# tyh666/News-Recommendation-MIND

Hardware: AMD Instinct MI355X
Metric: impressions/sec (train) + candidates scored/sec (eval), NRMS MIND-large 1/8 GPU (higher is better)
Workload: dtype f32; 1 GPU; NRMS train step: MHA news encoder + MHA user encoder, H=384, 12 heads, V=30522 word table (trainable), dropout 0.2, Adam; launch=hipGraph replay of the whole step, global_batch=32, per_gpu_batch=32, candidates=5, history=50, seq_len=30, parallelism=dp1

## Files before the change

include/newsrec_hip.h:

```cpp
#ifndef NEWSREC_HIP_H
#define NEWSREC_HIP_H

#include <stdint.h>

#ifdef __cplusplus
extern "C" {
#endif

typedef struct ihipStream_t* hipStream_t;

const char* nr_build_hash(void);


enum nr_rows_map {
  NR_ROWS_PLAIN = 0,
  NR_ROWS_GATHER = 1,
  NR_ROWS_CONV3 = 2
};

enum nr_layout {
  NR_KCONTIG = 0,
  NR_MNCONTIG = 1
};

// ... 134 lines not shown
                    int64_t ld_dout, float* dqk, int64_t ld_dqk, float* dv_out, int64_t ld_dv,
                    float* dbias_k, float* dbias_v, hipStream_t stream);

int nr_mha_pool_fwd(const float* y, int64_t ldy, const int64_t* yrows, const void* mask,
                    int32_t mask_dtype, int64_t nseq,
                    int32_t L, int32_t heads, int32_t dk, int32_t dv, const float* gamma,
                    const float* beta, float eps, float p_drop, uint64_t seed, uint64_t offset,
                    const uint64_t* rng, const float* q, float* news, int64_t ldn, float* zout,
                    int64_t ldz, float* oout, int64_t ldo, float* stats, float* probs,
                    int32_t prec, hipStream_t stream);

int nr_mha_pool_bwd(const float* y, int64_t ldy, const int64_t* yrows, const void* mask,
                    int32_t mask_dtype, int64_t nseq,
                    int32_t L, int32_t heads, int32_t dk, int32_t dv, const float* gamma,
                    const float* beta, float p_drop, uint64_t seed, uint64_t offset,
                    const uint64_t* rng, const float* q, const float* stats, const float* probs,
                    const float* dnews,
                    int64_t ldn, const float* dz, int64_t lddz, const float* o, int64_t ldo,
                    float* dob, int64_t lddob, float* dy, int64_t lddy,
                    float* dbias, float* dq, float* dgamma, float* dbeta, float* ws,
                    int32_t ws_copies, const int32_t* seg_off, int64_t dyu_row0, int64_t dy_rows,
                    uint32_t* dsto, int32_t prec, hipStream_t stream);


int nr_attn_pool_fwd(const float* x, int64_t ldx, const float* key, int64_t ldk, const float* q,
                     const void* mask, int32_t mask_dtype, const float* gamma, const float* beta,
                     float eps, float p_drop, uint64_t seed, uint64_t offset, const uint64_t* rng,
                     int64_t nseq, int32_t L, int32_t D, float scale, float* out, int64_t ldo,
                     float* zout,
                     int64_t ldz, float* stats, float* probs, hipStream_t stream);

int nr_attn_pool_bwd(const float* x, int64_t ldx, const float* key, int64_t ldk, const float* q,
                     const void* mask, int32_t mask_dtype, const float* gamma, const float* beta,
                     float p_drop, uint64_t seed, uint64_t offset, const uint64_t* rng,
                     int64_t nseq, int32_t L, int32_t D, float scale, const float* stats,
                     const float* probs,
                     const float* dout, int64_t lddo, const float* dz, int64_t lddz, float* dx,
                     int64_t lddx, float* dk, int64_t lddk, int32_t key_tanh, float* dq,
                     float* dgamma, float* dbeta, hipStream_t stream);

int nr_seq_pool_fwd(const float* x, int64_t ldx, const float* key, int64_t ldk, const float* q, int32_t qn,
                    const void* mask, int32_t mask_dtype, int64_t nseq, int32_t L, int32_t D, float scale,
                    float* out, int64_t ldo, float* probs, hipStream_t stream);

int nr_seq_pool_bwd(const float* x, int64_t ldx, const float* key, int64_t ldk, const float* q, int32_t qn,
                    const void* mask, int32_t mask_dtype, int64_t nseq, int32_t L, int32_t D, float scale,
// ... 248 lines not shown
```

news-recommendation-mind_amd/csrc/mha_pool.hip:

```cpp
#include "common.h"
#include "../../include/newsrec_hip.h"
#include <stdlib.h>

#include "mfma_planes.h"

namespace {

struct MPArgs {
  const float* y; int64_t ldy;
  const int64_t* yrows;
  const void* mask; int mask_dt;
  int64_t nseq; int L; int heads;
  float scale_attn, scale_pool;
  const float* gamma; const float* beta; float eps;
  float p_drop; uint64_t seed; uint64_t offset;
  uint32_t dkey, dthresh;
  const uint64_t* rng;
  const float* q;
  float* news; int64_t ldn;
  float* zout; int64_t ldz;
  float* stats; float* probs;
  const float* dz; int64_t lddz;
  float* dy; int64_t lddy;
  const int32_t* seg_off; int64_t dyu_row0;
// ... 41 lines not shown
__device__ __forceinline__ uint32_t row_byte_off(const MPArgs& g, int64_t tok) {
  return (uint32_t)((g.yrows ? g.yrows[tok] : tok) * g.ldy * 4);
}

__device__ __forceinline__ void stage_rows(const MPArgs& g, int64_t seq) {
  extern __shared__ uint32_t nr_mp_rows[];
  const int tid = threadIdx.x;
  if (tid < 32) nr_mp_rows[tid] = row_byte_off(g, seq * g.L + (tid < g.L ? tid : 0));
  __syncthreads();
}

__device__ __forceinline__ float drop_scale(const MPArgs& g, int64_t elem) {
  if (g.p_drop <= 0.f) return 1.f;
  return nr_dropout_keep(g.dkey, (uint32_t)elem, g.dthresh) ? 1.f / (1.f - g.p_drop) : 0.f;
}

__device__ __forceinline__ uint64_t token_bits(const MPArgs& g, int64_t seq) {
  const int lane = threadIdx.x & 63;
  const bool m = lane < g.L && nr_mask_at(g.mask, g.mask_dt, seq * g.L + lane);
  return __ballot(m);
}

template <int DK, int NP>
__device__ __forceinline__ void load_krow(const MPArgs& g, int64_t seq, int head, float (&a)[DK / 2]) {
  const int lane = threadIdx.x & 63, c = lane & 31, h = lane >> 5;
  constexpr int HK = DK / 2;
  if constexpr (NP > 0) {
    const bool ok = c < g.L;
    const float* kr = yrow(g, ok ? c : 0) + head * DK + 8 * h;
#pragma unroll
    for (int t = 0; t < DK / 16; ++t) {
#pragma unroll
      for (int q4 = 0; q4 < 2; ++q4) {
        const float4 v = *reinterpret_cast<const float4*>(kr + 16 * t + 4 * q4);
        float* d = a + 8 * t + 4 * q4;
        d[0] = ok ? v.x : 0.f; d[1] = ok ? v.y : 0.f; d[2] = ok ? v.z : 0.f; d[3] = ok ? v.w : 0.f;
      }
    }
  } else {
    const bool ok = c < g.L;
    const float* kr = yrow(g, ok ? c : 0) + head * DK + 4 * h;
#pragma unroll
    for (int s = 0; s < HK; s += 4) {
      const float4 v = *reinterpret_cast<const float4*>(kr + 2 * s);
      a[s] = ok ? v.x : 0.f; a[s + 1] = ok ? v.y : 0.f; a[s + 2] = ok ? v.z : 0.f; a[s + 3] = ok ? v.w : 0.f;
    }
  }
}

template <int DK, int NP>
__device__ __forceinline__ void stage_kblock(const float (&a)[DK / 2], int kb, float* tw) {
  const int lane = threadIdx.x & 63, c = lane & 31, h = lane >> 5;
  if constexpr (NP > 0) {
#pragma unroll
    for (int t = 2 * kb; t < 2 * kb + 2; ++t)
#pragma unroll
      for (int u = 0; u < 8; ++u) tw[c * 33 + 16 * t + 8 * h + u - 32 * kb] = a[8 * t + u];
  } else {
#pragma unroll
    for (int m = 4 * kb; m < 4 * kb + 4; ++m)
#pragma unroll
      for (int q = 0; q < 4; ++q) tw[c * 33 + 8 * m + 4 * h + q - 32 * kb] = a[4 * m + q];
  }
}

template <int DK, int NP>
__device__ __forceinline__ void head_probs_from(const MPArgs& g, uint64_t bits, const float (&a)[DK / 2],
                                                float (&p)[16]) {
  const int lane = threadIdx.x & 63, c = lane & 31, h = lane >> 5;
  constexpr int HK = DK / 2;
  f32x16 S;
#pragma unroll
  for (int r = 0; r < 16; ++r) S[r] = 0.f;
  if constexpr (NP == 0) {
#pragma unroll
    for (int s = 0; s < HK; ++s) S = __builtin_amdgcn_mfma_f32_32x32x2f32(a[s], a[s], S, 0, 0, 0);
  } else {
#pragma unroll
    for (int t = 0; t < DK / 16; ++t) {
      const Planes<NP> pk = planes8<NP>(a + 8 * t);
      mfma_x<NP>(S, pk, pk);
    }
  }
  const bool mj = (bits >> c) & 1ull;
  float mx = -INFINITY;
#pragma unroll
  for (int r = 0; r < 16; ++r) {
    const bool keep = mj && ((bits >> crow(r, h)) & 1ull);
    p[r] = keep ? S[r] * g.scale_attn : -INFINITY;
    mx = fmaxf(mx, p[r]);
  }
  mx = fmaxf(mx, __shfl_xor(mx, 32, 64));
// ... 243 lines not shown
      b += red[(ww * 3 + 1) * H + d];
      q += red[(ww * 3 + 2) * H + d];
    }
    atomicAdd(g.ws ? grad_slot(g, d) : &g.dgamma[d], a);
    atomicAdd(g.ws ? grad_slot(g, H + d) : &g.dbeta[d], b);
    atomicAdd(g.ws ? grad_slot(g, 2 * H + d) : &g.dq[d], q);
  }
  __syncthreads();
}

template <int DV>
struct DoSource {
  const float* base;
  int64_t ld;
  int L;
  bool global;
  __device__ __forceinline__ float at(int l, int col) const {
    if (!global) return base[l * ld + col];
    const float v = ld_off(base, 4u * (uint32_t)((l < L ? l : 0) * (int)ld + col));
    return l < L ? v : 0.f;
  }
};

template <int DK, int DV, int NP>
__device__ __forceinline__ void head_bwd(const MPArgs& g, int64_t seq, int head, uint64_t bits, float* tw,
                                         const DoSource<DV>& dO, float (&cs)[DV / 32 + DK / 32],
                                         const uint32_t* dsto) {
  const int lane = threadIdx.x & 63, c = lane & 31, h = lane >> 5;
  const int nq = g.heads * DK;

  float p[16];
  float ka[DK / 2];
  load_krow<DK, NP>(g, seq, head, ka);
  head_probs_from<DK, NP>(g, bits, ka, p);
  __builtin_amdgcn_sched_barrier(0);
  {
#pragma unroll
    for (int r = 0; r < 16; ++r) tw[c * 33 + crow(r, h)] = p[r];
    wave_lds_fence();
    float pt[16];
#pragma unroll
    for (int s = 0; s < 16; ++s) pt[s] = tw[crow(s, h) * 33 + c];
    wave_lds_fence();
#pragma unroll
    for (int vb = 0; vb < DV / 32; ++vb) {
      float bo[16];
#pragma unroll
      for (int s = 0; s < 16; ++s) bo[s] = dO.at(crow(s, h), vb * 32 + c);
      f32x16 acc;
#pragma unroll
      for (int r = 0; r < 16; ++r) acc[r] = 0.f;
      mfma16<NP>(acc, pt, bo);
      float sum = 0.f;
#pragma unroll
      for (int r = 0; r < 16; ++r) {
        const int i = crow(r, h);
        if (i < g.L && dsto[i] != ~0u) st_off(g.dy, dsto[i] + 4u * (uint32_t)(nq + head * DV + vb * 32 + c), acc[r]);
        sum += acc[r];
      }
      cs[vb] += sum;
      __builtin_amdgcn_sched_barrier(0);
    }
  }
  float dsv[16];
  {
    f32x16 dpt;
#pragma unroll
    for (int r = 0; r < 16; ++r) dpt[r] = 0.f;
    constexpr int HV = DV / 2;
    const bool rv = c < g.L;
    if constexpr (NP == 0) {
      const float* vrr = yrow(g, rv ? c : 0) + nq + head * DV + 4 * h;
#pragma unroll
      for (int s = 0; s < HV; s += 4) {
        float4 v4 = *reinterpret_cast<const float4*>(vrr + 2 * s);
        if (!rv) v4 = make_float4(0.f, 0.f, 0.f, 0.f);
        const int col = 4 * h + 2 * s;
        dpt = __builtin_amdgcn_mfma_f32_32x32x2f32(v4.x, dO.at(c, col), dpt, 0, 0, 0);
        dpt = __builtin_amdgcn_mfma_f32_32x32x2f32(v4.y, dO.at(c, col + 1), dpt, 0, 0, 0);
        dpt = __builtin_amdgcn_mfma_f32_32x32x2f32(v4.z, dO.at(c, col + 2), dpt, 0, 0, 0);
        dpt = __builtin_amdgcn_mfma_f32_32x32x2f32(v4.w, dO.at(c, col + 3), dpt, 0, 0, 0);
      }
    } else {
      const float* vrr = yrow(g, rv ? c : 0) + nq + head * DV + 8 * h;
#pragma unroll
      for (int t = 0; t < DV / 16; ++t) {
        float va[8], oa[8];
#pragma unroll
        for (int q4 = 0; q4 < 2; ++q4) {
          const float4 v4 = *reinterpret_cast<const float4*>(vrr + 16 * t + 4 * q4);
          va[4 * q4] = rv ? v4.x : 0.f; va[4 * q4 + 1] = rv ? v4.y : 0.f;
          va[4 * q4 + 2] = rv ? v4.z : 0.f; va[4 * q4 + 3] = rv ? v4.w : 0.f;
        }
#pragma unroll
        for (int u = 0; u < 8; ++u) oa[u] = dO.at(c, 16 * t + 8 * h + u);
        mfma_x<NP>(dpt, planes8<NP>(va), planes8<NP>(oa));
      }
    }
    float rs = 0.f;
#pragma unroll
    for (int r = 0; r < 16; ++r) rs = fmaf(p[r], dpt[r], rs);
    rs += __shfl_xor(rs, 32, 64);
#pragma unroll
    for (int r = 0; r < 16; ++r) dsv[r] = p[r] * (dpt[r] - rs) * g.scale_attn;
  }
  __builtin_amdgcn_sched_barrier(0);
#pragma unroll
  for (int r = 0; r < 16; ++r) tw[c * 33 + crow(r, h)] = dsv[r];
  wave_lds_fence();
#pragma unroll
  for (int r = 0; r < 16; ++r) dsv[r] += tw[crow(r, h) * 33 + c];
  wave_lds_fence();
#pragma unroll
  for (int kb = 0; kb < DK / 32; ++kb) {
    stage_kblock<DK, NP>(ka, kb, tw);
    wave_lds_fence();
    float bk[16];
#pragma unroll
    for (int s = 0; s < 16; ++s) bk[s] = tw[crow(s, h) * 33 + c];
    wave_lds_fence();
    f32x16 acc;
#pragma unroll
    for (int r = 0; r < 16; ++r) acc[r] = 0.f;
    mfma16<NP>(acc, dsv, bk);
    float sum = 0.f;
#pragma unroll
    for (int r = 0; r < 16; ++r) {
      const int j = crow(r, h);
      if (j < g.L && dsto[j] != ~0u) st_off(g.dy, dsto[j] + 4u * (uint32_t)(head * DK + kb * 32 + c), acc[r]);
      sum += acc[r];
    }
    cs[DV / 32 + kb] += sum;
    __builtin_amdgcn_sched_barrier(0);
  }
}

template <int DK, int DV>
__device__ __forceinline__ void flush_dbias(const MPArgs& g, int head, float (&cs)[DV / 32 + DK / 32]) {
  const int lane = threadIdx.x & 63, c = lane & 31, h = lane >> 5;
  const int nq = g.heads * DK;
#pragma unroll
  for (int i = 0; i < DV / 32 + DK / 32; ++i) {
    const float v = cs[i] + __shfl_xor(cs[i], 32, 64);
    const int col = i < DV / 32 ? nq + head * DV + i * 32 + c : head * DK + (i - DV / 32) * 32 + c;
    if (h == 0) atomicAdd(g.ws ? grad_slot(g, 3 * (int64_t)g.heads * DV + col) : &g.dbias[col], v);
    cs[i] = 0.f;
  }
}

template <int DK, int DV, int NH64, int NP, bool SAVED>
__global__ __launch_bounds__(384) void mha_pool_bwd_kernel(MPArgs g) {
  if (g.rng) g.dkey = nr_dropout_key(g.rng[0], g.rng[1] + g.offset);
  extern __shared__ __attribute__((aligned(16))) float sm[];
  constexpr int H = NH64 * 64;
  constexpr int SO = H + 1;
  const int nw = blockDim.x >> 6;
  float* os = sm + 32;
// ... 135 lines not shown
    if (lane == 0) {
      float4* rc = reinterpret_cast<float4*>(g.dob + row * g.lddob);
      rc[0] = make_float4(g.stats[2 * row], rstd, sg, sgx);
      rc[1] = make_float4(dsl, pl, 0.f, 0.f);
    }
  }
#pragma unroll
  for (int k = 0; k < NH64; ++k) {
    red[w][0][lane + 64 * k] = dgam[k];
    red[w][1][lane + 64 * k] = dbet[k];
    red[w][2][lane + 64 * k] = dqp[k];
  }
  __syncthreads();
  float* ogam = g.ws ? grad_slot(g, 0) : g.dgamma;
  float* obet = g.ws ? grad_slot(g, H) : g.dbeta;
  float* oq = g.ws ? grad_slot(g, 2 * H) : g.dq;
  for (int d = tid; d < H; d += 256) {
    atomicAdd(&ogam[d], (red[0][0][d] + red[1][0][d]) + (red[2][0][d] + red[3][0][d]));
    atomicAdd(&obet[d], (red[0][1][d] + red[1][1][d]) + (red[2][1][d] + red[3][1][d]));
    atomicAdd(&oq[d], (red[0][2][d] + red[1][2][d]) + (red[2][2][d] + red[3][2][d]));
  }
}

constexpr int HB_TITLES = 1;

template <int DK, int DV, int NP>
__global__ __launch_bounds__(256, 4) void mha_head_bwd_kernel(MPArgs g) {
  if (g.rng) g.dkey = nr_dropout_key(g.rng[0], g.rng[1] + g.offset);
  extern __shared__ __attribute__((aligned(16))) float sm[];
  const int lane = threadIdx.x & 63, w = threadIdx.x >> 6, nw = blockDim.x >> 6;
  const int head = blockIdx.y * nw + w;
  if (head >= g.heads) return;
  uint32_t* rows = reinterpret_cast<uint32_t*>(sm) + 32 * w;
  uint32_t* dsts = reinterpret_cast<uint32_t*>(sm) + 32 * nw + 32 * w;
  float* tw = sm + 64 * nw + w * 32 * 33;
  float* dot = sm + 64 * nw + nw * 32 * 33 + w * 32 * (DV + 1);
  float cs[DV / 32 + DK / 32];
#pragma unroll
  for (int i = 0; i < DV / 32 + DK / 32; ++i) cs[i] = 0.f;
  const int64_t s0 = (int64_t)blockIdx.x * HB_TITLES;
#pragma unroll 1
  for (int64_t seq = s0; seq < s0 + HB_TITLES && seq < g.nseq; ++seq) {
    const uint32_t roff = lane < 32 ? row_byte_off(g, seq * g.L + (lane < g.L ? lane : 0)) : 0u;
    const uint64_t bits = token_bits(g, seq);
    uint32_t doff = ~0u;
    if (lane < g.L) doff = g.dsto ? g.dsto[seq * g.L + lane] : (uint32_t)((seq * g.L + lane) * g.lddy * 4);
    constexpr int F4 = DV / 4;
    constexpr int PER = 32 * F4 / 64;
    static_assert(64 % F4 == 0, "a lane keeps its four columns in every row it loads");
    float4 v[PER], ra[PER], rb[PER];
    const int col0 = head * DV + 4 * (lane % F4);
    {
      const float* src = g.o + (seq * g.L) * g.ldo + head * DV;
#pragma unroll
      for (int i = 0; i < PER; ++i) {
        const int e = lane + 64 * i, r = e / F4, c4 = e % F4;
        const int rr = r < g.L ? r : 0;
        v[i] = *reinterpret_cast<const float4*>(
            reinterpret_cast<const char*>(src) + 4u * (uint32_t)(rr * (int)g.ldo + 4 * c4));
        const float4* rc = reinterpret_cast<const float4*>(g.dob + (seq * g.L + rr) * g.lddob);
        ra[i] = rc[0];
        rb[i] = rc[1];
      }
    }
    float gm[4], qd[4], dn[4];
#pragma unroll
    for (int j = 0; j < 4; ++j) {
      gm[j] = g.gamma[col0 + j];
      qd[j] = g.q[col0 + j];
      dn[j] = g.news[seq * g.ldn + col0 + j];
    }
    {
      const bool drop = g.p_drop > 0.f;
      const float dsc = drop ? 1.f / (1.f - g.p_drop) : 1.f;
      const uint32_t Hc = (uint32_t)(g.heads * DV);
#pragma unroll
      for (int i = 0; i < PER; ++i) {
        const int r = (lane + 64 * i) / F4;
        const int64_t row = seq * g.L + (r < g.L ? r : 0);
        float o[4] = {v[i].x, v[i].y, v[i].z, v[i].w}, d[4];
#pragma unroll
        for (int j = 0; j < 4; ++j) {
          const uint32_t col = (uint32_t)(col0 + j);
          const bool keep = !drop || nr_dropout_keep(g.dkey, (uint32_t)row * Hc + col, g.dthresh);
          const float dzv = g.dz ? g.dz[row * g.lddz + col] : 0.f;
          const float xh = (o[j] - ra[i].x) * ra[i].y;
          d[j] = ln_row_dO(xh, ra[i].y, ra[i].z, ra[i].w, rb[i].y, rb[i].x, dn[j], qd[j], gm[j], dzv,
                           keep ? dsc : 0.f);
        }
        v[i] = r < g.L ? make_float4(d[0], d[1], d[2], d[3]) : make_float4(0.f, 0.f, 0.f, 0.f);
      }
    }
    if (lane < 32) {
      rows[lane] = roff;
      dsts[lane] = doff;
    }
#pragma unroll
    for (int i = 0; i < PER; ++i) {
      const int e = lane + 64 * i, r = e / F4, c4 = e % F4;
      float* d = dot + r * (DV + 1) + 4 * c4;
      d[0] = v[i].x; d[1] = v[i].y; d[2] = v[i].z; d[3] = v[i].w;
    }
    wave_lds_fence();
    DoSource<DV> dO{dot, DV + 1, g.L, false};
    head_bwd<DK, DV, NP>(g, seq, head, bits, tw, dO, cs, dsts);
    wave_lds_fence();
  }
  flush_dbias<DK, DV>(g, head, cs);
}

__global__ __launch_bounds__(64) void copies_reduce_kernel(MPArgs g, int H, int NY) {
  const int i = blockIdx.x * 64 + threadIdx.x;
  if (i >= 3 * H + NY) return;
  float s = 0.f;
  for (int c0 = 0; c0 < g.ws_copies; c0 += 16) {
    float v[16];
#pragma unroll
    for (int c = 0; c < 16; ++c) v[c] = c0 + c < g.ws_copies ? g.ws[(int64_t)(c0 + c) * g.ws_ld + i] : 0.f;
#pragma unroll
    for (int c = 0; c < 16; ++c) {
      s += v[c];
      if (c0 + c < g.ws_copies) g.ws[(int64_t)(c0 + c) * g.ws_ld + i] = 0.f;
    }
  }
  float* out = i < H ? g.dgamma + i : i < 2 * H ? g.dbeta + (i - H) : i < 3 * H ? g.dq + (i - 2 * H) : g.dbias + (i - 3 * H);
  *out += s;
}

size_t fwd_smem(int H) { return (size_t)(32 + 32 * (H + 1) + 32) * sizeof(float); }
size_t bwd_smem(int H, int nw) {
  const size_t tiles = (size_t)nw * 32 * 33, red = (size_t)nw * 3 * H;
  return (size_t)(32 + 32 * (H + 1) + 32 + 32 + 64 + 2 * 32 * (H / 64) + (tiles > red ? tiles : red)) * sizeof(float);
}

size_t head_bwd_smem(int nw, int dv) { return (size_t)(64 * nw + nw * 32 * 33 + nw * 32 * (dv + 1)) * sizeof(float); }

enum Pass { FWD = 0, BWD_FUSED = 1, BWD_SPLIT = 2 };

template <typename K>
void allow_smem(K kern, size_t sz) {
  if (sz > 64 * 1024) (void)hipFuncSetAttribute((const void*)kern, hipFuncAttributeMaxDynamicSharedMemorySize, (int)sz);
}

template <int DK, int NP>
__device__ __forceinline__ void load_krow64(const MPArgs& g, int head, int rb, float (&a)[DK / 2]) {
  const int lane = threadIdx.x & 63, c = lane & 31, h = lane >> 5;
  const int row = c + 32 * rb;
  const bool ok = row < g.L;
  if constexpr (NP > 0) {
    const float* kr = yrow(g, ok ? row : 0) + head * DK + 8 * h;
#pragma unroll
    for (int t = 0; t < DK / 16; ++t)
#pragma unroll
      for (int q4 = 0; q4 < 2; ++q4) {
        const float4 v = *reinterpret_cast<const float4*>(kr + 16 * t + 4 * q4);
        float* d = a + 8 * t + 4 * q4;
        d[0] = ok ? v.x : 0.f; d[1] = ok ? v.y : 0.f; d[2] = ok ? v.z : 0.f; d[3] = ok ? v.w : 0.f;
      }
  } else {
    const float* kr = yrow(g, ok ? row : 0) + head * DK + 4 * h;
// ... 132 lines not shown

size_t user_pool_smem(int H, int L) { return (size_t)(64 + L * (H + 1) + 64) * sizeof(float); }
constexpr size_t NR_MAX_LDS = 160 * 1024;

template <int DK, int DV, int NH64>
int launch_user_pool(const MPArgs& g, hipStream_t s) {
  const size_t sz = user_pool_smem(NH64 * 64, g.L);
  const int nw = g.heads < 4 ? 4 : g.heads;
  if (g.np == 3) {
    allow_smem(mha_user_pool_fwd_kernel<DK, DV, NH64, 3>, sz);
    hipLaunchKernelGGL((mha_user_pool_fwd_kernel<DK, DV, NH64, 3>), dim3((unsigned)g.nseq), dim3(64 * nw), sz, s, g);
  } else if (g.np == 1) {
    allow_smem(mha_user_pool_fwd_kernel<DK, DV, NH64, 1>, sz);
    hipLaunchKernelGGL((mha_user_pool_fwd_kernel<DK, DV, NH64, 1>), dim3((unsigned)g.nseq), dim3(64 * nw), sz, s, g);
  } else {
    allow_smem(mha_user_pool_fwd_kernel<DK, DV, NH64, 0>, sz);
    hipLaunchKernelGGL((mha_user_pool_fwd_kernel<DK, DV, NH64, 0>), dim3((unsigned)g.nseq), dim3(64 * nw), sz, s, g);
  }
  NR_LAUNCH_CHECK();
  return NR_OK;
}

template <int DK, int DV, int NH64, int NP>
int launch_np(const MPArgs& g, Pass pass, hipStream_t s) {
  const int H = NH64 * 64;
  if (pass == FWD) {
    const int nw = 4;
    const size_t sz = fwd_smem(H);
    allow_smem(mha_pool_fwd_kernel<DK, DV, NH64, NP>, sz);
    hipLaunchKernelGGL((mha_pool_fwd_kernel<DK, DV, NH64, NP>), dim3((unsigned)g.nseq), dim3(64 * nw), sz, s, g);
  } else if (pass == BWD_FUSED) {
    const int nw = (g.heads + 1) / 2 < 4 ? 4 : (g.heads + 1) / 2;
    const size_t sz = bwd_smem(H, nw);
    if (g.o) {
      allow_smem(mha_pool_bwd_kernel<DK, DV, NH64, NP, true>, sz);
      hipLaunchKernelGGL((mha_pool_bwd_kernel<DK, DV, NH64, NP, true>), dim3((unsigned)g.nseq), dim3(64 * nw), sz,
                         s, g);
    } else {
      allow_smem(mha_pool_bwd_kernel<DK, DV, NH64, NP, false>, sz);
      hipLaunchKernelGGL((mha_pool_bwd_kernel<DK, DV, NH64, NP, false>), dim3((unsigned)g.nseq), dim3(64 * nw), sz,
                         s, g);
    }
    if (g.ws) {
      const int NY = g.heads * (DK + DV);
      hipLaunchKernelGGL(copies_reduce_kernel, dim3((unsigned)((3 * H + NY + 63) / 64)), dim3(64), 0, s, g, H, NY);
    }
  } else {
    hipLaunchKernelGGL((mha_ln_bwd_kernel<NH64>), dim3((unsigned)g.nseq), dim3(256), 0, s, g);
    MPArgs g2 = g;
    g2.rows_per_wave = 1;
    const unsigned gx = (unsigned)((g.nseq + HB_TITLES - 1) / HB_TITLES), gy = (unsigned)((g.heads + 3) / 4);
    hipLaunchKernelGGL((mha_head_bwd_kernel<DK, DV, NP>), dim3(gx, gy), dim3(256), head_bwd_smem(4, DV), s, g2);
    if (g.ws) {
      const int NY = g.heads * (DK + DV);
      hipLaunchKernelGGL(copies_reduce_kernel, dim3((unsigned)((3 * H + NY + 63) / 64)), dim3(64), 0, s, g, H, NY);
    }
  }
  NR_LAUNCH_CHECK();
  return NR_OK;
}

template <int DK, int DV, int NH64>
int launch(const MPArgs& g, Pass pass, hipStream_t s) {
  if (g.np == 3) return launch_np<DK, DV, NH64, 3>(g, pass, s);
  if (g.np == 1) return launch_np<DK, DV, NH64, 1>(g, pass, s);
  return launch_np<DK, DV, NH64, 0>(g, pass, s);
}

int dispatch(const MPArgs& g, int dk, int dv, Pass pass, hipStream_t s) {
  const int H = g.heads * dv;
  if (H % 64) return NR_EINVAL(9);
  const int nh64 = H / 64;
#define NR_CASE(K, V, N) \
  if (dk == K && dv == V && nh64 == N) return launch<K, V, N>(g, pass, s);
  NR_CASE(64, 32, 6)
  NR_CASE(64, 64, 12)
  NR_CASE(64, 32, 4)
  NR_CASE(32, 32, 6)
#undef NR_CASE
  return NR_EINVAL(8);
}

bool al16(const void* p) { return (reinterpret_cast<uintptr_t>(p) & 15) == 0; }

}

extern "C" int nr_mha_pool_fwd(const float* y, int64_t ldy, const int64_t* yrows, const void* mask,
                               int32_t mask_dtype, int64_t nseq,
                               int32_t L, int32_t heads, int32_t dk, int32_t dv, const float* gamma,
                               const float* beta, float eps, float p_drop, uint64_t seed, uint64_t offset, const uint64_t* rng,
                               const float* q, float* news, int64_t ldn, float* zout, int64_t ldz, float* oout,
                               int64_t ldo, float* stats, float* probs, int32_t prec, hipStream_t stream) {
  if (L < 1 || L > 32 || heads < 1 || heads > 12) return NR_EINVAL(0);
  if (prec != NR_GEMM_F32 && prec != NR_GEMM_BF16X6 && prec != NR_GEMM_BF16) return NR_EINVAL(4);
  if (!y || !mask || !gamma || !beta || !q || !news || !stats || !probs) return NR_EINVAL(1);
  if ((ldy & 3) || !al16(y)) return NR_EINVAL(2);
  if (nseq == 0) return NR_OK;
// ... 50 lines not shown
    return NR_EINVAL(1);
  if (dy_rows < nseq * L || dy_rows * lddy * 4 >= ((int64_t)1 << 32)) return NR_EINVAL(6);
  if (seg_off && (!yrows || !dsto || dyu_row0 < nseq * L || dyu_row0 > dy_rows)) return NR_EINVAL(7);
  if ((ldy & 3) || !al16(y)) return NR_EINVAL(2);
  if (nseq == 0) return NR_OK;
  MPArgs g{};
  g.y = y; g.ldy = ldy; g.yrows = yrows; g.mask = mask; g.mask_dt = mask_dtype; g.nseq = nseq; g.L = L; g.heads = heads;
  g.scale_attn = 1.0f / sqrtf((float)dk); g.scale_pool = 1.0f / sqrtf((float)(heads * dv));
  g.gamma = gamma; g.beta = beta; g.p_drop = p_drop; g.seed = seed; g.offset = offset;
  g.dkey = nr_dropout_key(seed, offset); g.dthresh = nr_dropout_threshold(p_drop); g.rng = rng; g.q = q;
  g.news = const_cast<float*>(dnews); g.ldn = ldn; g.stats = const_cast<float*>(stats);
  g.probs = const_cast<float*>(probs); g.dz = dz; g.lddz = lddz; g.dy = dy; g.lddy = lddy; g.dbias = dbias;
  g.dq = dq; g.dgamma = dgamma; g.dbeta = dbeta;
  g.o = const_cast<float*>(o); g.ldo = ldo; g.dob = dob; g.lddob = lddob;
  g.seg_off = seg_off; g.dyu_row0 = dyu_row0; g.dsto = seg_off ? dsto : nullptr;
  if (o && ((dob && (lddob < 8 || (lddob & 3) || !al16(dob))) || ldo < (int64_t)heads * dv || (ldo & 3) || !al16(o)))
    return NR_EINVAL(3);
  g.np = prec == NR_GEMM_BF16 ? 1 : 0;
  if (ws && (!o || ws_copies < 1 || ws_copies > 1024)) return NR_EINVAL(5);
  g.ws = ws; g.ws_copies = ws_copies;
  g.ws_ld = ((int64_t)3 * heads * dv + (int64_t)heads * (dk + dv) + 3) & ~int64_t(3);
  return dispatch(g, dk, dv, o && dob ? BWD_SPLIT : BWD_FUSED, stream);
}
```

news-recommendation-mind_amd/newsrec_amd/_lib.py:

```python
import ctypes
import os

import torch

_HERE = os.path.dirname(os.path.abspath(__file__))
LIB_PATH = os.environ.get("NR_LIB_PATH") or os.path.join(_HERE, "lib", "libnewsrec_hip.so")

c_f32p = ctypes.c_void_p
c_i64 = ctypes.c_int64
c_i32 = ctypes.c_int32
c_f32 = ctypes.c_float
c_u64 = ctypes.c_uint64
c_ptr = ctypes.c_void_p

ROWS_PLAIN, ROWS_GATHER, ROWS_CONV3 = 0, 1, 2
KCONTIG, MNCONTIG = 0, 1
EPI_STORE, EPI_STORE_RELU, EPI_ATOMIC, EPI_SCATTER = 0, 1, 2, 3
MASK_U8, MASK_I64, MASK_F64, MASK_F32 = 0, 1, 2, 3
EPI_STORE_TANH, EPI_ACCUM_GATE, EPI_ACCUM, EPI_SCATTER_STORE = 4, 5, 6, 7
EPI_STORE_GELU, EPI_GELU_GRAD, EPI_SCATTER_ZEROED = 8, 9, 10
GEMM_F32, GEMM_BF16X6, GEMM_BF16 = 0, 1, 2
CELL_LSTM, CELL_GRU = 0, 1
SCORE_RAW, SCORE_LOG_SOFTMAX, SCORE_SIGMOID = 0, 1, 2

# ... 78 lines not shown
                     c_ptr, c_i64, c_ptr],
    "nr_birnn_bwd": [c_ptr, c_ptr, c_i64, c_i32, c_i32, c_ptr, c_i64, c_ptr, c_i64, c_ptr, c_i64, c_ptr],
    "nr_score_fwd": [c_ptr, c_i64, c_ptr, c_ptr, c_i64, c_i64, c_i32, c_i32, c_i32, c_ptr, c_ptr],
    "nr_score_bwd": [c_ptr, c_i64, c_ptr, c_i64, c_ptr, c_ptr, c_i64, c_i32, c_i32, c_i32, c_ptr, c_i64, c_ptr,
                     c_i64, c_ptr],
    "nr_adam": [c_ptr, c_ptr, c_ptr, c_ptr, c_i64, c_f32, c_f32, c_f32, c_f32, c_f32, c_i64, c_ptr, c_f32, c_ptr],
    "nr_embedding_fwd": [c_ptr, c_i64, c_i64, c_ptr, c_i64, c_ptr, c_ptr],
    "nr_embedding_bwd": [c_ptr, c_i64, c_i64, c_ptr, c_i64, c_i64, c_ptr, c_ptr],
    "nr_rows_add_ordered": [c_ptr, c_i64, c_i64, c_i64, c_ptr, c_i64, c_i64, c_ptr, c_i64, c_ptr],
    "nr_transpose_f32": [c_ptr, c_i64, c_i64, c_i64, c_ptr, c_i64, c_ptr],
    "nr_xsoftmax_fwd": [c_ptr, c_ptr, c_i32, c_i64, c_i64, c_ptr, c_ptr],
    "nr_xsoftmax_bwd": [c_ptr, c_ptr, c_i64, c_i64, c_ptr, c_ptr],
    "nr_gather_rows_f32": [c_ptr, c_i64, c_i64, c_ptr, c_i64, c_i64, c_ptr, c_i64, c_ptr],
    "nr_colsum": [c_ptr, c_i64, c_i64, c_i64, c_ptr, c_ptr, c_ptr],
    "nr_colsum_ws": [c_ptr, c_i64, c_i64, c_i64, c_ptr, c_ptr, c_ptr, c_ptr],
    "nr_colsum_workspace": [c_i64, c_i64],
    "nr_mha_pool_fwd": [c_ptr, c_i64, c_ptr, c_ptr, c_i32, c_i64, c_i32, c_i32, c_i32, c_i32, c_ptr, c_ptr, c_f32, c_f32,
                        c_u64, c_u64, c_ptr, c_ptr, c_ptr, c_i64, c_ptr, c_i64, c_ptr, c_i64, c_ptr, c_ptr, c_i32,
                        c_ptr],
    "nr_mha_pool_bwd": [c_ptr, c_i64, c_ptr, c_ptr, c_i32, c_i64, c_i32, c_i32, c_i32, c_i32, c_ptr, c_ptr, c_f32, c_u64,
                        c_u64, c_ptr, c_ptr, c_ptr, c_ptr, c_ptr, c_i64, c_ptr, c_i64, c_ptr, c_i64, c_ptr, c_i64,
                        c_ptr, c_i64, c_ptr, c_ptr, c_ptr, c_ptr, c_ptr, c_i32, c_ptr, c_i64, c_i64, c_ptr,
                        c_i32, c_ptr],
    "nr_form_train_batch": [c_ptr, c_i64, c_ptr, c_i64, c_ptr, c_ptr, c_ptr, c_ptr, c_ptr, c_ptr, c_ptr, c_i64,
                            c_i32, c_i32, c_i32, c_i32, c_u64, c_u64, c_ptr, c_ptr, c_ptr, c_ptr, c_ptr, c_ptr,
                            c_ptr, c_ptr, c_ptr, c_ptr, c_ptr, c_ptr, c_ptr],
    "nr_rng_take": [c_ptr, c_ptr, c_u64, c_ptr],
    "nr_form_eval_batch": [c_i64, c_i64, c_ptr, c_i64, c_ptr, c_ptr, c_ptr, c_ptr, c_ptr, c_i64, c_i32, c_i32,
                           c_i32, c_ptr, c_ptr, c_ptr, c_ptr, c_ptr, c_ptr, c_ptr, c_ptr],
    "nr_gather_news_rows": [c_ptr, c_i64, c_ptr, c_ptr, c_i64, c_i32, c_ptr, c_ptr, c_ptr, c_ptr],
    "nr_score_ragged": [c_ptr, c_i64, c_i64, c_ptr, c_ptr, c_i64, c_i64, c_ptr, c_i64, c_i64, c_i32, c_i32, c_ptr,
                        c_ptr, c_ptr],
    "nr_impression_metrics": [c_ptr, c_ptr, c_ptr, c_i64, c_ptr, c_i32, c_ptr, c_ptr, c_ptr],
    "nr_rank_ordinal": [c_ptr, c_ptr, c_i64, c_i64, c_i64, c_ptr, c_ptr, c_ptr, c_ptr],
    "nr_format_prediction": [c_ptr, c_ptr, c_ptr, c_i64, c_i64, c_ptr, c_i64, c_ptr],
    "nr_topk_workspace": [c_i64, c_i64, c_i32, c_i32],
    "nr_topk_news": [c_ptr, c_i64, c_i64, c_ptr, c_i64, c_i64, c_i32, c_i32, c_i64, c_ptr, c_ptr, c_i32, c_i32, c_ptr,
                     c_ptr, c_ptr, c_i64, c_ptr, c_ptr],
    "nr_bm25_count": [c_ptr, c_i64, c_i64, c_i32, c_i32, c_i32, c_i32, c_i32, c_ptr, c_ptr, c_ptr, c_ptr],
    "nr_bm25_build_workspace": [c_i64, c_i32, c_i32],
    "nr_bm25_build": [c_ptr, c_i64, c_i64, c_i32, c_i32, c_i32, c_i32, c_i32, c_i32, c_i32, c_ptr, c_ptr, c_ptr, c_ptr,
                      c_ptr, c_i64, c_ptr],
    "nr_bm25_forward": [c_ptr, c_i64, c_i64, c_i32, c_i32, c_i32, c_ptr, c_ptr, c_ptr, c_i64, c_ptr, c_ptr],
    "nr_bm25_topk_workspace": [c_i64, c_i64, c_i32, c_i32],
    "nr_bm25_topk": [c_ptr, c_i64, c_i64, c_i32, c_ptr, c_i64, c_ptr, c_i64, c_ptr, c_i64, c_i32, c_i32, c_i32, c_i32,
                     c_i32, c_i32, c_i64, c_ptr, c_ptr, c_i32, c_i32, c_ptr, c_ptr, c_ptr, c_i64, c_ptr],
# ... 130 lines not shown
```

Baseline: 25230 impressions/s.

## Make MHA head backward a persistent grid with prefetched next-sequence indices

The per-head backward kernel now launches a grid capped at the resident workgroup count and walks sequences with a grid stride, instead of one block per title. While working on one sequence it loads the next sequence's row offsets, scatter targets and mask bits, then stages them in LDS. It also preloads V rows into registers, stages the per-row LN stats through LDS instead of redundant per-lane loads, and reorders the dS phase before the dV phase. This trades launch and tail overhead plus index-load latency for more register and LDS pressure and an occupancy query. A small exported helper reports the walk cap.

Result: faster. 25740 impressions/s (median of 6 runs) (+2.0%).

```diff
diff --git a/include/newsrec_hip.h b/include/newsrec_hip.h
--- a/include/newsrec_hip.h
+++ b/include/newsrec_hip.h
@@ -180,6 +180,8 @@
                     int32_t ws_copies, const int32_t* seg_off, int64_t dyu_row0, int64_t dy_rows,
                     uint32_t* dsto, int32_t prec, hipStream_t stream);
 
+int nr_mha_pool_walk_workgroups(int32_t pass, int32_t heads, int32_t dk, int32_t dv, int32_t prec);
+
 
 int nr_attn_pool_fwd(const float* x, int64_t ldx, const float* key, int64_t ldk, const float* q,
                      const void* mask, int32_t mask_dtype, const float* gamma, const float* beta,
diff --git a/news-recommendation-mind_amd/csrc/mha_pool.hip b/news-recommendation-mind_amd/csrc/mha_pool.hip
--- a/news-recommendation-mind_amd/csrc/mha_pool.hip
+++ b/news-recommendation-mind_amd/csrc/mha_pool.hip
@@ -87,8 +87,9 @@
 }
 
 template <int DK, int NP>
-__device__ __forceinline__ void load_krow(const MPArgs& g, int64_t seq, int head, float (&a)[DK / 2]) {
-  const int lane = threadIdx.x & 63, c = lane & 31, h = lane >> 5;
+__device__ __forceinline__ void load_krow(const MPArgs& g, int64_t seq, int head, float (&a)[DK / 2],
+                                          int lane = threadIdx.x & 63) {
+  const int c = lane & 31, h = lane >> 5;
   constexpr int HK = DK / 2;
   if constexpr (NP > 0) {
     const bool ok = c < g.L;
@@ -114,8 +115,9 @@
 }
 
 template <int DK, int NP>
-__device__ __forceinline__ void stage_kblock(const float (&a)[DK / 2], int kb, float* tw) {
-  const int lane = threadIdx.x & 63, c = lane & 31, h = lane >> 5;
+__device__ __forceinline__ void stage_kblock(const float (&a)[DK / 2], int kb, float* tw,
+                                             int lane = threadIdx.x & 63) {
+  const int c = lane & 31, h = lane >> 5;
   if constexpr (NP > 0) {
 #pragma unroll
     for (int t = 2 * kb; t < 2 * kb + 2; ++t)
@@ -131,8 +133,8 @@
 
 template <int DK, int NP>
 __device__ __forceinline__ void head_probs_from(const MPArgs& g, uint64_t bits, const float (&a)[DK / 2],
-                                                float (&p)[16]) {
-  const int lane = threadIdx.x & 63, c = lane & 31, h = lane >> 5;
+                                                float (&p)[16], int lane = threadIdx.x & 63) {
+  const int c = lane & 31, h = lane >> 5;
   constexpr int HK = DK / 2;
   f32x16 S;
 #pragma unroll
@@ -422,22 +424,17 @@
   }
 };
 
-template <int DK, int DV, int NP>
-__device__ __forceinline__ void head_bwd(const MPArgs& g, int64_t seq, int head, uint64_t bits, float* tw,
-                                         const DoSource<DV>& dO, float (&cs)[DV / 32 + DK / 32],
-                                         const uint32_t* dsto) {
-  const int lane = threadIdx.x & 63, c = lane & 31, h = lane >> 5;
+template <int DK, int DV, int NP, bool VPRE, bool WALK>
+__device__ __forceinline__ void head_bwd_from(const MPArgs& g, int head, const float (&ka)[DK / 2],
+                                              const float (&vr)[DV / 2], const float (&p)[16], float* tw,
+                                              const DoSource<DV>& dO, float (&cs)[DV / 32 + DK / 32],
+                                              const uint32_t* dsto, int lane = threadIdx.x & 63) {
+  const int c = lane & 31, h = lane >> 5;
   const int nq = g.heads * DK;
-
-  float p[16];
-  float ka[DK / 2];
-  load_krow<DK, NP>(g, seq, head, ka);
-  head_probs_from<DK, NP>(g, bits, ka, p);
-  __builtin_amdgcn_sched_barrier(0);
-  {
-#pragma unroll
-    for (int r = 0; r < 16; ++r) tw[c * 33 + crow(r, h)] = p[r];
-    wave_lds_fence();
+#pragma unroll
+  for (int r = 0; r < 16; ++r) tw[c * 33 + crow(r, h)] = p[r];
+  wave_lds_fence();
+  auto dv_phase = [&]() {
     float pt[16];
 #pragma unroll
     for (int s = 0; s < 16; ++s) pt[s] = tw[crow(s, h) * 33 + c];
@@ -461,9 +458,9 @@
       cs[vb] += sum;
       __builtin_amdgcn_sched_barrier(0);
     }
-  }
+  };
   float dsv[16];
-  {
+  auto ds_phase = [&]() {
     f32x16 dpt;
 #pragma unroll
     for (int r = 0; r < 16; ++r) dpt[r] = 0.f;
@@ -473,8 +470,13 @@
       const float* vrr = yrow(g, rv ? c : 0) + nq + head * DV + 4 * h;
 #pragma unroll
       for (int s = 0; s < HV; s += 4) {
-        float4 v4 = *reinterpret_cast<const float4*>(vrr + 2 * s);
-        if (!rv) v4 = make_float4(0.f, 0.f, 0.f, 0.f);
+        float4 v4;
+        if constexpr (VPRE) {
+          v4 = make_float4(vr[s], vr[s + 1], vr[s + 2], vr[s + 3]);
+        } else {
+          v4 = *reinterpret_cast<const float4*>(vrr + 2 * s);
+          if (!rv) v4 = make_float4(0.f, 0.f, 0.f, 0.f);
+        }
         const int col = 4 * h + 2 * s;
         dpt = __builtin_amdgcn_mfma_f32_32x32x2f32(v4.x, dO.at(c, col), dpt, 0, 0, 0);
         dpt = __builtin_amdgcn_mfma_f32_32x32x2f32(v4.y, dO.at(c, col + 1), dpt, 0, 0, 0);
@@ -486,23 +488,39 @@
 #pragma unroll
       for (int t = 0; t < DV / 16; ++t) {
         float va[8], oa[8];
-#pragma unroll
-        for (int q4 = 0; q4 < 2; ++q4) {
-          const float4 v4 = *reinterpret_cast<const float4*>(vrr + 16 * t + 4 * q4);
-          va[4 * q4] = rv ? v4.x : 0.f; va[4 * q4 + 1] = rv ? v4.y : 0.f;
-          va[4 * q4 + 2] = rv ? v4.z : 0.f; va[4 * q4 + 3] = rv ? v4.w : 0.f;
+        if constexpr (VPRE) {
+#pragma unroll
+          for (int u = 0; u < 8; ++u) va[u] = vr[8 * t + u];
+        } else {
+#pragma unroll
+          for (int q4 = 0; q4 < 2; ++q4) {
+            const float4 v4 = *reinterpret_cast<const float4*>(vrr + 16 * t + 4 * q4);
+            va[4 * q4] = rv ? v4.x : 0.f; va[4 * q4 + 1] = rv ? v4.y : 0.f;
+            va[4 * q4 + 2] = rv ? v4.z : 0.f; va[4 * q4 + 3] = rv ? v4.w : 0.f;
+          }
         }
 #pragma unroll
         for (int u = 0; u < 8; ++u) oa[u] = dO.at(c, 16 * t + 8 * h + u);
         mfma_x<NP>(dpt, planes8<NP>(va), planes8<NP>(oa));
       }
     }
+    float pr[16];
+#pragma unroll
+    for (int r = 0; r < 16; ++r) pr[r] = WALK ? tw[c * 33 + crow(r, h)] : p[r];
     float rs = 0.f;
 #pragma unroll
-    for (int r = 0; r < 16; ++r) rs = fmaf(p[r], dpt[r], rs);
+    for (int r = 0; r < 16; ++r) rs = fmaf(pr[r], dpt[r], rs);
     rs += __shfl_xor(rs, 32, 64);
 #pragma unroll
-    for (int r = 0; r < 16; ++r) dsv[r] = p[r] * (dpt[r] - rs) * g.scale_attn;
+    for (int r = 0; r < 16; ++r) dsv[r] = pr[r] * (dpt[r] - rs) * g.scale_attn;
+  };
+  if constexpr (WALK) {
+    ds_phase();
+    __builtin_amdgcn_sched_barrier(0);
+    dv_phase();
+  } else {
+    dv_phase();
+    ds_phase();
   }
   __builtin_amdgcn_sched_barrier(0);
 #pragma unroll
@@ -513,7 +531,7 @@
   wave_lds_fence();
 #pragma unroll
   for (int kb = 0; kb < DK / 32; ++kb) {
-    stage_kblock<DK, NP>(ka, kb, tw);
+    stage_kblock<DK, NP>(ka, kb, tw, lane);
     wave_lds_fence();
     float bk[16];
 #pragma unroll
@@ -533,6 +551,19 @@
     cs[DV / 32 + kb] += sum;
     __builtin_amdgcn_sched_barrier(0);
   }
+}
+
+template <int DK, int DV, int NP>
+__device__ __forceinline__ void head_bwd(const MPArgs& g, int64_t seq, int head, uint64_t bits, float* tw,
+                                         const DoSource<DV>& dO, float (&cs)[DV / 32 + DK / 32],
+                                         const uint32_t* dsto) {
+  float p[16];
+  float ka[DK / 2];
+  load_krow<DK, NP>(g, seq, head, ka);
+  head_probs_from<DK, NP>(g, bits, ka, p);
+  __builtin_amdgcn_sched_barrier(0);
+  const float none[DV / 2] = {};
+  head_bwd_from<DK, DV, NP, false, false>(g, head, ka, none, p, tw, dO, cs, dsto);
 }
 
 template <int DK, int DV>
@@ -714,33 +745,106 @@
   }
 }
 
-constexpr int HB_TITLES = 1;
+constexpr int HB_STAGE = 65;
+
+struct HbIndex { uint32_t yr, ds, mb, m0, m1; };
+
+__device__ __forceinline__ HbIndex hb_index_load(const MPArgs& g, int seq, int lane) {
+  const int l = lane & 31;
+  const uint32_t t = (uint32_t)(seq * g.L + (l < g.L ? l : 0));
+  const char* safe = reinterpret_cast<const char*>(g.y);
+  const auto word = [](const char* base, uint32_t off) { return *reinterpret_cast<const uint32_t*>(base + off); };
+  HbIndex ix;
+  ix.yr = word(g.yrows ? reinterpret_cast<const char*>(g.yrows) : safe, g.yrows ? 8u * t : 0u);
+  ix.ds = word(g.dsto ? reinterpret_cast<const char*>(g.dsto) : safe, g.dsto ? 4u * t : 0u);
+  const uint32_t es = g.mask_dt == NR_MASK_U8 ? 1u : g.mask_dt == NR_MASK_F32 ? 4u : 8u;
+  const char* mask = reinterpret_cast<const char*>(g.mask);
+  ix.mb = *reinterpret_cast<const uint8_t*>(mask + es * t);
+  ix.m0 = word(es == 1 ? safe : mask, es == 1 ? 0u : es * t);
+  ix.m1 = word(es == 1 ? safe : mask, es == 1 ? 0u : es * t + (es == 8 ? 4u : 0u));
+  return ix;
+}
+
+__device__ __forceinline__ void hb_index_stage(const MPArgs& g, int seq, const HbIndex& ix, uint32_t* stg,
+                                               int lane) {
+  const int l = lane & 31;
+  const uint32_t t = (uint32_t)(seq * g.L + (l < g.L ? l : 0));
+  const uint32_t roff = (g.yrows ? ix.yr : t) * (uint32_t)(g.ldy * 4);
+  uint32_t doff = g.dsto ? ix.ds : t * (uint32_t)(g.lddy * 4);
+  if (l >= g.L) doff = ~0u;
+  stg[lane] = lane < 32 ? roff : doff;
+  const bool m = g.mask_dt == NR_MASK_U8    ? ix.mb != 0
+                 : g.mask_dt == NR_MASK_I64 ? (ix.m0 | ix.m1) != 0
+                 : g.mask_dt == NR_MASK_F64 ? (ix.m0 | (ix.m1 & 0x7fffffffu)) != 0
+                                            : (ix.m0 & 0x7fffffffu) != 0;
+  const uint64_t bits = __ballot(lane < g.L && m);
+  if (lane == 0) stg[64] = (uint32_t)bits;
+}
+
+__device__ __forceinline__ uint64_t hb_index_promote(const uint32_t* stg, uint32_t* rows, uint32_t* dsts,
+                                                    int lane) {
+  const uint32_t v = stg[lane];
+  const uint32_t b = stg[64];
+  (lane < 32 ? rows : dsts - 32)[lane] = v;
+  wave_lds_fence();
+  return (uint64_t)(uint32_t)__builtin_amdgcn_readfirstlane((int)b);
+}
+
+template <int DK, int DV, int NP>
+__device__ __forceinline__ void load_vrow(const MPArgs& g, int head, float (&vr)[DV / 2], int lane) {
+  const int c = lane & 31, h = lane >> 5;
+  const bool ok = c < g.L;
+  const float* vrr = yrow(g, ok ? c : 0) + g.heads * DK + head * DV;
+  if constexpr (NP == 0) {
+#pragma unroll
+    for (int s = 0; s < DV / 2; s += 4) {
+      const float4 v = *reinterpret_cast<const float4*>(vrr + 4 * h + 2 * s);
+      vr[s] = ok ? v.x : 0.f; vr[s + 1] = ok ? v.y : 0.f; vr[s + 2] = ok ? v.z : 0.f; vr[s + 3] = ok ? v.w : 0.f;
+    }
+  } else {
+#pragma unroll
+    for (int t = 0; t < DV / 16; ++t)
+#pragma unroll
+      for (int q4 = 0; q4 < 2; ++q4) {
+        const float4 v = *reinterpret_cast<const float4*>(vrr + 8 * h + 16 * t + 4 * q4);
+        float* d = vr + 8 * t + 4 * q4;
+        d[0] = ok ? v.x : 0.f; d[1] = ok ? v.y : 0.f; d[2] = ok ? v.z : 0.f; d[3] = ok ? v.w : 0.f;
+      }
+  }
+}
 
 template <int DK, int DV, int NP>
 __global__ __launch_bounds__(256, 4) void mha_head_bwd_kernel(MPArgs g) {
   if (g.rng) g.dkey = nr_dropout_key(g.rng[0], g.rng[1] + g.offset);
   extern __shared__ __attribute__((aligned(16))) float sm[];
-  const int lane = threadIdx.x & 63, w = threadIdx.x >> 6, nw = blockDim.x >> 6;
+  const int w = __builtin_amdgcn_readfirstlane(threadIdx.x >> 6), nw = blockDim.x >> 6;
   const int head = blockIdx.y * nw + w;
   if (head >= g.heads) return;
   uint32_t* rows = reinterpret_cast<uint32_t*>(sm) + 32 * w;
   uint32_t* dsts = reinterpret_cast<uint32_t*>(sm) + 32 * nw + 32 * w;
   float* tw = sm + 64 * nw + w * 32 * 33;
   float* dot = sm + 64 * nw + nw * 32 * 33 + w * 32 * (DV + 1);
+  uint32_t* stg = reinterpret_cast<uint32_t*>(sm) + 64 * nw + nw * 32 * 33 + nw * 32 * (DV + 1) + HB_STAGE * w;
   float cs[DV / 32 + DK / 32];
 #pragma unroll
   for (int i = 0; i < DV / 32 + DK / 32; ++i) cs[i] = 0.f;
-  const int64_t s0 = (int64_t)blockIdx.x * HB_TITLES;
+  const int G = gridDim.x, nseq = (int)g.nseq;
+  int seq0 = blockIdx.x;
+  hb_index_stage(g, seq0, hb_index_load(g, seq0, threadIdx.x & 63), stg, threadIdx.x & 63);
+  wave_lds_fence();
 #pragma unroll 1
-  for (int64_t seq = s0; seq < s0 + HB_TITLES && seq < g.nseq; ++seq) {
-    const uint32_t roff = lane < 32 ? row_byte_off(g, seq * g.L + (lane < g.L ? lane : 0)) : 0u;
-    const uint64_t bits = token_bits(g, seq);
-    uint32_t doff = ~0u;
-    if (lane < g.L) doff = g.dsto ? g.dsto[seq * g.L + lane] : (uint32_t)((seq * g.L + lane) * g.lddy * 4);
+  for (; seq0 < nseq; seq0 += G) {
+    const int64_t seq = seq0;
+    int lane = threadIdx.x & 63;
+    asm volatile("" : "+v"(lane));
+    const int c = lane & 31, h = lane >> 5;
+    const uint64_t bits = hb_index_promote(stg, rows, dsts, lane);
+    const int nxt = seq0 + G < nseq ? seq0 + G : nseq - 1;
+    const HbIndex nix = hb_index_load(g, nxt, lane);
     constexpr int F4 = DV / 4;
     constexpr int PER = 32 * F4 / 64;
     static_assert(64 % F4 == 0, "a lane keeps its four columns in every row it loads");
-    float4 v[PER], ra[PER], rb[PER];
+    float4 v[PER];
     const int col0 = head * DV + 4 * (lane % F4);
     {
       const float* src = g.o + (seq * g.L) * g.ldo + head * DV;
@@ -750,11 +854,9 @@
         const int rr = r < g.L ? r : 0;
         v[i] = *reinterpret_cast<const float4*>(
             reinterpret_cast<const char*>(src) + 4u * (uint32_t)(rr * (int)g.ldo + 4 * c4));
-        const float4* rc = reinterpret_cast<const float4*>(g.dob + (seq * g.L + rr) * g.lddob);
-        ra[i] = rc[0];
-        rb[i] = rc[1];
       }
     }
+    const float4 rt = reinterpret_cast<const float4*>(g.dob + (seq * g.L + (c < g.L ? c : 0)) * g.lddob)[h];
     float gm[4], qd[4], dn[4];
 #pragma unroll
     for (int j = 0; j < 4; ++j) {
@@ -762,6 +864,10 @@
       qd[j] = g.q[col0 + j];
       dn[j] = g.news[seq * g.ldn + col0 + j];
     }
+    float ka[DK / 2], vr[DV / 2];
+    load_krow<DK, NP>(g, seq, head, ka, lane);
+    *reinterpret_cast<float4*>(tw + 8 * c + 4 * h) = rt;
+    wave_lds_fence();
     {
       const bool drop = g.p_drop > 0.f;
       const float dsc = drop ? 1.f / (1.f - g.p_drop) : 1.f;
@@ -769,23 +875,21 @@
 #pragma unroll
       for (int i = 0; i < PER; ++i) {
         const int r = (lane + 64 * i) / F4;
-        const int64_t row = seq * g.L + (r < g.L ? r : 0);
+        const int rr = r < g.L ? r : 0;
+        const int64_t row = seq * g.L + rr;
+        const float4 ra = *reinterpret_cast<const float4*>(tw + 8 * rr);
+        const float2 rb = *reinterpret_cast<const float2*>(tw + 8 * rr + 4);
         float o[4] = {v[i].x, v[i].y, v[i].z, v[i].w}, d[4];
 #pragma unroll
         for (int j = 0; j < 4; ++j) {
           const uint32_t col = (uint32_t)(col0 + j);
           const bool keep = !drop || nr_dropout_keep(g.dkey, (uint32_t)row * Hc + col, g.dthresh);
           const float dzv = g.dz ? g.dz[row * g.lddz + col] : 0.f;
-          const float xh = (o[j] - ra[i].x) * ra[i].y;
-          d[j] = ln_row_dO(xh, ra[i].y, ra[i].z, ra[i].w, rb[i].y, rb[i].x, dn[j], qd[j], gm[j], dzv,
-                           keep ? dsc : 0.f);
+          const float xh = (o[j] - ra.x) * ra.y;
+          d[j] = ln_row_dO(xh, ra.y, ra.z, ra.w, rb.y, rb.x, dn[j], qd[j], gm[j], dzv, keep ? dsc : 0.f);
         }
         v[i] = r < g.L ? make_float4(d[0], d[1], d[2], d[3]) : make_float4(0.f, 0.f, 0.f, 0.f);
       }
-    }
-    if (lane < 32) {
-      rows[lane] = roff;
-      dsts[lane] = doff;
     }
 #pragma unroll
     for (int i = 0; i < PER; ++i) {
@@ -793,9 +897,14 @@
       float* d = dot + r * (DV + 1) + 4 * c4;
       d[0] = v[i].x; d[1] = v[i].y; d[2] = v[i].z; d[3] = v[i].w;
     }
+    hb_index_stage(g, nxt, nix, stg, lane);
     wave_lds_fence();
     DoSource<DV> dO{dot, DV + 1, g.L, false};
-    head_bwd<DK, DV, NP>(g, seq, head, bits, tw, dO, cs, dsts);
+    load_vrow<DK, DV, NP>(g, head, vr, lane);
+    float p[16];
+    head_probs_from<DK, NP>(g, bits, ka, p, lane);
+    __builtin_amdgcn_sched_barrier(0);
+    head_bwd_from<DK, DV, NP, true, true>(g, head, ka, vr, p, tw, dO, cs, dsts, lane);
     wave_lds_fence();
   }
   flush_dbias<DK, DV>(g, head, cs);
@@ -825,9 +934,32 @@
   return (size_t)(32 + 32 * (H + 1) + 32 + 32 + 64 + 2 * 32 * (H / 64) + (tiles > red ? tiles : red)) * sizeof(float);
 }
 
-size_t head_bwd_smem(int nw, int dv) { return (size_t)(64 * nw + nw * 32 * 33 + nw * 32 * (dv + 1)) * sizeof(float); }
+size_t head_bwd_smem(int nw, int dv) {
+  return (size_t)(64 * nw + nw * 32 * 33 + nw * 32 * (dv + 1) + nw * HB_STAGE) * sizeof(float);
+}
 
 enum Pass { FWD = 0, BWD_FUSED = 1, BWD_SPLIT = 2 };
+
+template <typename Kern>
+int resident_workgroups(Kern kern, int threads, size_t smem) {
+  static int cache[16] = {0};
+  int dev = 0;
+  if (hipGetDevice(&dev) != hipSuccess || dev < 0 || dev >= 16) dev = 0;
+  if (cache[dev] == 0) {
+    int cus = 0, per = 0;
+    if (hipDeviceGetAttribute(&cus, hipDeviceAttributeMultiprocessorCount, dev) != hipSuccess || cus < 1) cus = 1;
+    if (hipOccupancyMaxActiveBlocksPerMultiprocessor(&per, kern, threads, smem) != hipSuccess || per < 1) per = 1;
+    cache[dev] = cus * per;
+  }
+  return cache[dev];
+}
+
+template <int DK, int DV, int NP>
+int head_walk_cap(int heads) {
+  const int gy = (heads + 3) / 4;
+  const int n = resident_workgroups(mha_head_bwd_kernel<DK, DV, NP>, 256, head_bwd_smem(4, DV)) / gy;
+  return n < 1 ? 1 : n;
+}
 
 template <typename K>
 void allow_smem(K kern, size_t sz) {
@@ -1006,8 +1138,12 @@
 }
 
 template <int DK, int DV, int NH64, int NP>
-int launch_np(const MPArgs& g, Pass pass, hipStream_t s) {
+int launch_np(const MPArgs& g, Pass pass, hipStream_t s, int* walk) {
   const int H = NH64 * 64;
+  if (walk) {
+    *walk = pass == BWD_SPLIT ? head_walk_cap<DK, DV, NP>(g.heads) : 0;
+    return NR_OK;
+  }
   if (pass == FWD) {
     const int nw = 4;
     const size_t sz = fwd_smem(H);
@@ -1033,7 +1169,8 @@
     hipLaunchKernelGGL((mha_ln_bwd_kernel<NH64>), dim3((unsigned)g.nseq), dim3(256), 0, s, g);
     MPArgs g2 = g;
     g2.rows_per_wave = 1;
-    const unsigned gx = (unsigned)((g.nseq + HB_TITLES - 1) / HB_TITLES), gy = (unsigned)((g.heads + 3) / 4);
+    const int64_t cap = head_walk_cap<DK, DV, NP>(g.heads);
+    const unsigned gx = (unsigned)(g.nseq < cap ? g.nseq : cap), gy = (unsigned)((g.heads + 3) / 4);
     hipLaunchKernelGGL((mha_head_bwd_kernel<DK, DV, NP>), dim3(gx, gy), dim3(256), head_bwd_smem(4, DV), s, g2);
     if (g.ws) {
       const int NY = g.heads * (DK + DV);
@@ -1045,18 +1182,18 @@
 }
 
 template <int DK, int DV, int NH64>
-int launch(const MPArgs& g, Pass pass, hipStream_t s) {
-  if (g.np == 3) return launch_np<DK, DV, NH64, 3>(g, pass, s);
-  if (g.np == 1) return launch_np<DK, DV, NH64, 1>(g, pass, s);
-  return launch_np<DK, DV, NH64, 0>(g, pass, s);
-}
-
-int dispatch(const MPArgs& g, int dk, int dv, Pass pass, hipStream_t s) {
+int launch(const MPArgs& g, Pass pass, hipStream_t s, int* walk) {
+  if (g.np == 3) return launch_np<DK, DV, NH64, 3>(g, pass, s, walk);
+  if (g.np == 1) return launch_np<DK, DV, NH64, 1>(g, pass, s, walk);
+  return launch_np<DK, DV, NH64, 0>(g, pass, s, walk);
+}
+
+int dispatch(const MPArgs& g, int dk, int dv, Pass pass, hipStream_t s, int* walk = nullptr) {
   const int H = g.heads * dv;
   if (H % 64) return NR_EINVAL(9);
   const int nh64 = H / 64;
 #define NR_CASE(K, V, N) \
-  if (dk == K && dv == V && nh64 == N) return launch<K, V, N>(g, pass, s);
+  if (dk == K && dv == V && nh64 == N) return launch<K, V, N>(g, pass, s, walk);
   NR_CASE(64, 32, 6)
   NR_CASE(64, 64, 12)
   NR_CASE(64, 32, 4)
@@ -1153,3 +1290,15 @@
   g.ws_ld = ((int64_t)3 * heads * dv + (int64_t)heads * (dk + dv) + 3) & ~int64_t(3);
   return dispatch(g, dk, dv, o && dob ? BWD_SPLIT : BWD_FUSED, stream);
 }
+
+extern "C" int nr_mha_pool_walk_workgroups(int32_t pass, int32_t heads, int32_t dk, int32_t dv, int32_t prec) {
+  if (heads < 1 || heads > 12) return NR_EINVAL(0);
+  if (prec != NR_GEMM_F32 && prec != NR_GEMM_BF16X6 && prec != NR_GEMM_BF16) return NR_EINVAL(4);
+  if (pass != FWD && pass != BWD_FUSED && pass != BWD_SPLIT) return NR_EINVAL(1);
+  MPArgs g{};
+  g.heads = heads;
+  g.np = prec == NR_GEMM_BF16 ? 1 : prec == NR_GEMM_BF16X6 && pass == FWD ? 3 : 0;
+  int walk = 0;
+  const int rc = dispatch(g, dk, dv, (Pass)pass, nullptr, &walk);
+  return rc != NR_OK ? rc : walk;
+}
diff --git a/news-recommendation-mind_amd/newsrec_amd/_lib.py b/news-recommendation-mind_amd/newsrec_amd/_lib.py
--- a/news-recommendation-mind_amd/newsrec_amd/_lib.py
+++ b/news-recommendation-mind_amd/newsrec_amd/_lib.py
@@ -124,6 +124,7 @@
                         c_u64, c_ptr, c_ptr, c_ptr, c_ptr, c_ptr, c_i64, c_ptr, c_i64, c_ptr, c_i64, c_ptr, c_i64,
                         c_ptr, c_i64, c_ptr, c_ptr, c_ptr, c_ptr, c_ptr, c_i32, c_ptr, c_i64, c_i64, c_ptr,
                         c_i32, c_ptr],
+    "nr_mha_pool_walk_workgroups": [c_i32, c_i32, c_i32, c_i32, c_i32],
     "nr_form_train_batch": [c_ptr, c_i64, c_ptr, c_i64, c_ptr, c_ptr, c_ptr, c_ptr, c_ptr, c_ptr, c_ptr, c_i64,
                             c_i32, c_i32, c_i32, c_i32, c_u64, c_u64, c_ptr, c_ptr, c_ptr, c_ptr, c_ptr, c_ptr,
                             c_ptr, c_ptr, c_ptr, c_ptr, c_ptr, c_ptr, c_ptr],
```
